# aswanthabam/JPEG_Decoder

Measured on AMD Instinct MI355X. Metric: Mpixels/s decoded (IDCT+colour), higher is better.
Workload: dtype f32; 1 GPU; stream of 4096x4096 baseline 4:4:4 images, 32 images per step (one launch) per GPU, coefficient blocks resident in HBM; sampling=4:4:4, parallelism=images sharded x1, no collective, launched_by=bench.py

## Files before the change

### jpeg_decoder_amd/csrc/jb_huff.hip

```cpp
#include <hip/hip_runtime.h>
#include <stdint.h>

#include "jb_huff_core.h"
#include "jb_kernels.h"

extern __shared__ __attribute__((aligned(16))) uint8_t lds[];

namespace {

constexpr uint32_t L = kJbhLanes;
constexpr int kMaxPasses = (int)L + 4;

__constant__ uint8_t kZz2Dev[64] = {0,   2,   16,  32,  18,  4,   6,   20,  34,  48, 64,  50,  36,  22,  8,   10,
                                    24,  38,  52,  66,  80,  96,  82,  68,  54,  40, 26,  12,  14,  28,  42,  56,
                                    70,  84,  98,  112, 114, 100, 86,  72,  58,  44, 30,  46,  60,  74,  88,  102,
                                    116, 118, 104, 90,  76,  62,  78,  92,  106, 120, 122, 108, 94,  110, 124, 126};

struct Misc {
  uint32_t *w;
  static constexpr uint32_t kBytes = 256u, kZz2 = 0u, kZz2Words = 64u / 4u, kScan = 16u, kScanWords = L / 64u * 5u, kFold = 40u, kFoldWords = 8u;
  static_assert(kZz2 + kZz2Words <= kScan && kScan + kScanWords <= kFold && (kFold + kFoldWords) * 4u <= kBytes, "sub-areas: disjoint, inside the 256 bytes");
  __device__ uint32_t *zz2() const { return w + kZz2; }
  __device__ uint32_t *scan() const { return w + kScan; }
  __device__ uint32_t *fold() const { return w + kFold; }
};
template <uint32_t kMaxChunk>
struct Lay {
  static constexpr uint32_t kRows = jbh_rows(kMaxChunk);
  static constexpr uint32_t kNcp = kMaxChunk * 8u / kJbCheckpointBits;
  static_assert(kNcp <= kJbCheckpoints, "records per chunk");
  static constexpr uint32_t off_cp = kRows * L * 4u;
  static constexpr uint32_t off_xbit = off_cp + kNcp * L * 4u;
  static constexpr uint32_t off_xmeta = off_xbit + L * 4u;
  static constexpr uint32_t off_misc = off_xmeta + L * 4u;
  static constexpr uint32_t off_tab = off_misc + Misc::kBytes;
  static constexpr uint32_t bytes(uint32_t n_tabs) { return off_tab + n_tabs * kJbT1Entries * 2u + kJbT2Tables * kJbT2Entries * 2u; }
  static __device__ uint32_t *stream() { return (uint32_t *)lds; }
  static __device__ uint32_t *cp() { return (uint32_t *)(lds + off_cp); }
  static __device__ uint32_t *xbit() { return (uint32_t *)(lds + off_xbit); }
  static __device__ uint32_t *xmeta() { return (uint32_t *)(lds + off_xmeta); }
  static __device__ Misc misc() { return Misc{(uint32_t *)(lds + off_misc)}; }
  static __device__ uint16_t *tab() { return (uint16_t *)(lds + off_tab); }
};
static_assert(Lay<64>::bytes(2) == 30976 && Lay<64>::bytes(3) == 33024 && Lay<64>::bytes(4) == 35072 && Lay<64>::bytes(5) == 37120 && Lay<64>::bytes(6) == 39168, "LDS bytes: 1.1 KiB more per workgroup cost a third of the waves (NOTES.md)");
static_assert(Lay<128>::bytes(2) == 49408 && Lay<128>::bytes(3) == 51456 && Lay<128>::bytes(4) == 53504 && Lay<128>::bytes(5) == 55552 && Lay<128>::bytes(6) == 57600, "LDS bytes");

struct LaneId {
  uint32_t ci;
  bool owned, active;
  uint32_t gidx;
  uint32_t start, end;
  uint32_t seg;
  bool first, last;
  uint32_t u0, u_end;
};
__device__ __forceinline__ LaneId lane_id(const JbHuffLaunch &p, const JbHuffImage &img, const JbHuffWg &wg, uint32_t tid, uint32_t warm, bool warm_go) {
  LaneId x;
  x.ci = wg.first_chunk + tid - warm;
  const bool has = tid < warm + kJbOwnChunks && x.ci < img.n_chunks;
  x.owned = tid >= warm && has;
  x.active = has && (x.owned || warm_go);
  x.gidx = img.state_off + (has ? x.ci : img.n_chunks - 1u);
  const JbChunkDesc cd = p.chunks[x.gidx];
  x.seg = cd.seg & 0x7fffffffu;
  x.first = (cd.seg >> 31) != 0;
  uint32_t seg_end = p.starts[img.int_off + x.seg + 1];
  if (seg_end > img.scan_len) seg_end = img.scan_len;
  x.start = cd.start < seg_end ? cd.start : seg_end;
  x.end = x.start + img.chunk_bytes < seg_end ? x.start + img.chunk_bytes : seg_end;
  x.last = x.end == seg_end;
  x.u0 = jbh_u_of_bit(x.start, x.start * 8u), x.u_end = x.u0 + (x.end - x.start) * 8u;
  return x;
}

template <uint32_t kRows>
__device__ __forceinline__ void load_stream(uint32_t *stream, const uint8_t *img_scan, uint32_t start, uint32_t tid) {
  const uint8_t *src = img_scan + (int32_t)jbh_base_byte(start);
#pragma unroll
  for (uint32_t q = 0; q < (kRows + 3u) / 4u; q++) {
    const uint4 v = *(const uint4 *)(src + 16u * q);
    const uint32_t d[4] = {v.x, v.y, v.z, v.w};
#pragma unroll
    for (uint32_t i = 0; i < 4; i++)
      if (4u * q + i < kRows) stream[(4u * q + i) * L + tid] = __builtin_bswap32(d[i]);
  }
}

__device__ __forceinline__ void load_tables(uint16_t *tab, const JbHuffLaunch &p, const JbHuffImage &img, uint32_t tid) {
  const JbHuffTables *set = p.tables + img.table_set;
  const uint4 *s1 = (const uint4 *)set->t1;
  uint4 *d = (uint4 *)tab;
  const uint32_t n1 = img.n_tabs * kJbT1Entries * 2u / 16u;
  for (uint32_t i = tid; i < n1; i += L) d[i] = s1[i];
  const uint4 *s2 = (const uint4 *)set->t2;
  constexpr uint32_t n2 = kJbT2Tables * kJbT2Entries * 2u / 16u;
  for (uint32_t i = tid; i < n2; i += L) d[n1 + i] = s2[i];
}

struct Seg {
  uint32_t f, n, d0, d1, d2;
};
__device__ __forceinline__ Seg seg_combine(const Seg &a, const Seg &b) {
  Seg r;
  r.f = a.f | b.f;
  r.n = b.f ? b.n : a.n + b.n;
  r.d0 = b.f ? b.d0 : a.d0 + b.d0;
  r.d1 = b.f ? b.d1 : a.d1 + b.d1;
  r.d2 = b.f ? b.d2 : a.d2 + b.d2;
  return r;
}
__device__ __forceinline__ Seg seg_shfl_up(const Seg &x, int off) {
  Seg r;
  r.f = __shfl_up(x.f, off);
  r.n = __shfl_up(x.n, off);
  r.d0 = __shfl_up(x.d0, off);
  r.d1 = __shfl_up(x.d1, off);
  r.d2 = __shfl_up(x.d2, off);
  return r;
}
__device__ __forceinline__ void seg_store(uint32_t *s, const Seg &x) { s[0] = x.f, s[1] = x.n, s[2] = x.d0, s[3] = x.d1, s[4] = x.d2; }
__device__ __forceinline__ Seg seg_load(const uint32_t *s) { return Seg{s[0], s[1], s[2], s[3], s[4]}; }
__device__ __forceinline__ Seg seg_scan_wg(Seg x, uint32_t *scratch, uint32_t tid, Seg *total) {
  const uint32_t lane = tid & 63u, wave = tid >> 6;
#pragma unroll
  for (int off = 1; off < 64; off <<= 1) {
    const Seg t = seg_shfl_up(x, off);
    if (lane >= (uint32_t)off) x = seg_combine(t, x);
  }
  __syncthreads();
  if (lane == 63u) seg_store(scratch + wave * 5u, x);
  __syncthreads();
  Seg run{0, 0, 0, 0, 0};
  Seg all{0, 0, 0, 0, 0};
#pragma unroll
  for (uint32_t w = 0; w < L / 64u; w++) {
    const Seg t = seg_load(scratch + w * 5u);
    if (w < wave) run = seg_combine(run, t);
    all = seg_combine(all, t);
  }
  *total = all;
  return seg_combine(run, x);
}

__device__ __forceinline__ Seg seg_left_workgroups(const JbHuffLaunch &p, const JbHuffImage &img, const JbHuffWg &wg, const Misc &misc, uint32_t tid) {
  const uint32_t w_first = img.wg0, w_me = img.wg0 + wg.first_chunk / kJbOwnChunks;
  uint32_t *const red = misc.fold();
  if (tid < 8) red[tid] = 0;
  __syncthreads();
  uint32_t last_f = 0;
  for (uint32_t w = w_first + tid; w < w_me; w += L)
    if (p.wgsum[w].has_first) last_f = w - w_first + 1u;
  if (last_f) atomicMax(&red[0], last_f);
  __syncthreads();
  const uint32_t from = red[0];
  uint32_t a_n = 0, a0 = 0, a1 = 0, a2 = 0;
  for (uint32_t w = w_first + tid; w < w_me; w += L) {
    if (w - w_first + 1u >= from) {
      const JbWgSum s = p.wgsum[w];
      a_n += s.blocks, a0 += s.dc[0], a1 += s.dc[1], a2 += s.dc[2];
    }
  }
  if (a_n) atomicAdd(&red[1], a_n);
  if (a0) atomicAdd(&red[2], a0);
  if (a1) atomicAdd(&red[3], a1);
  if (a2) atomicAdd(&red[4], a2);
  __syncthreads();
  return Seg{from ? 1u : 0u, red[1], red[2], red[3], red[4]};
}
__device__ __forceinline__ Seg seg_left_lanes(const Seg &mine, const Misc &misc, uint32_t tid) {
  Seg total;
  const Seg incl = seg_scan_wg(mine, misc.scan(), tid, &total);
  Seg left = seg_shfl_up(incl, 1);
  if ((tid & 63u) == 0) {
    left = Seg{0, 0, 0, 0, 0};
    for (uint32_t w = 0; w < (tid >> 6); w++) left = seg_combine(left, seg_load(misc.scan() + w * 5u));
  }
  return left;
}
__device__ __forceinline__ JbWgSum *wgsum_of(const JbHuffLaunch &p, const JbHuffImage &img, const JbHuffWg &wg) { return p.wgsum + img.wg0 + wg.first_chunk / kJbOwnChunks; }

}

template <uint32_t kMaxChunk>
__global__ __launch_bounds__(kJbHuffLanes) void jb_huff_sync_kernel(const JbHuffLaunch p, const int launch) {
  using Ly = Lay<kMaxChunk>;
  uint32_t *const xbit = Ly::xbit(), *const xmeta = Ly::xmeta();
  const uint32_t tid = threadIdx.x;
  const JbHuffWg wg = p.sync_wgs[blockIdx.x];
  const JbHuffImage img = p.images[wg.image];
  const LaneId me = lane_id(p, img, wg, tid, kJbWarmChunks, launch == 0);
  const size_t n_all = p.n_chunks_total;

  JbChunkState entry{me.start * 8u, 0u}, exitst{0u, 0u};
  bool changed = me.active;
  if (launch > 0) {
    bool c0 = false;
    JbChunkState ne{0u, 0u};
    if (tid == kJbWarmChunks && me.owned && !me.first) {
      ne = p.exit[me.gidx - 1u];
      c0 = !jbh_same_state(ne, p.entry[me.gidx]);
    }
    if (!__syncthreads_or(c0)) return;
    entry = p.entry[me.gidx];
    exitst = p.exit[me.gidx];
    changed = c0;
    if (c0) entry = jbh_entry_from_exit(ne);
  }
  load_tables(Ly::tab(), p, img, tid);
  if (me.active) load_stream<Ly::kRows>(Ly::stream(), p.scan + img.scan_off, me.start, tid);
  uint32_t *const cpl = Ly::cp() + tid;
#pragma unroll
  for (uint32_t i = 0; i < Ly::kNcp; i++) cpl[i * L] = launch > 0 ? p.cps[i * n_all + me.gidx] : kJbhCpNone;
  __syncthreads();
  const JbhCtx cx = jbh_ctx(Ly::stream() + tid, Ly::tab(), nullptr, img);

  for (int pass = 0; pass < kMaxPasses; pass++) {
    if (__builtin_amdgcn_ballot_w64(changed) != 0) {
      JbhLane st = jbh_lane_from(entry, me.start, me.u_end, cx.nb4, changed);
      uint32_t none = 0;
      while (st.u < me.u_end) {
        const uint32_t up = st.u;
        (void)jbh_step<false>(cx, st, none, none, none, nullptr, 0u);
        if (((st.u ^ up) >> 8) != 0) {
          uint32_t *rec = cpl + ((st.u >> 8) - 1u) * L;
          const uint32_t s = jbh_pack_state(st), old = *rec;
          const bool met = (st.u < me.u_end) & jbh_cp_same_place(old, s);
          *rec = met ? old : s;
          st.u = met ? jbh_met_at((st.u >> 8) - 1u) : st.u;
        }
      }
      JBH_TRACE_PASS_END(pass);
      if (changed) {
        if (jbh_has_met(st.u)) {
          const uint32_t met_i = jbh_met_checkpoint(st.u);
          const uint32_t dn = st.nblk - jbh_cp_blocks(cpl[met_i * L]);
          for (uint32_t i = met_i; i < Ly::kNcp; i++) cpl[i * L] = jbh_cp_add_blocks(cpl[i * L], dn);
          exitst.meta = jbh_meta_add_blocks(exitst.meta, dn);
        } else {
          exitst = JbChunkState{jbh_bit_of_u(me.start, st.u), jbh_exit_meta(st)};
        }
      }
    }
    xbit[tid] = exitst.bitpos;
    xmeta[tid] = jbh_meta_state(exitst.meta);
    __syncthreads();
    changed = false;
    if (me.active && !me.first && tid > (launch == 0 ? 0u : kJbWarmChunks)) {
      const uint32_t nbit = xbit[tid - 1u], nmeta = xmeta[tid - 1u];
      if (nbit != entry.bitpos || nmeta != jbh_meta_state(entry.meta)) {
        entry = JbChunkState{nbit, nmeta};
        changed = true;
      }
    }
    if (!__syncthreads_or(changed)) break;
  }
  if (me.owned) {
    p.entry[me.gidx] = entry;
    p.exit[me.gidx] = exitst;
#pragma unroll
    for (uint32_t i = 0; i < Ly::kNcp; i++) p.cps[i * n_all + me.gidx] = cpl[i * L];
  }
  Seg mine{0, 0, 0, 0, 0};
  if (me.owned) {
    mine.f = me.first ? 1u : 0u;
    mine.n = jbh_meta_blocks(exitst.meta) + (me.first ? me.seg * img.ri * img.nb : 0u);
  }
  Seg total;
  (void)seg_scan_wg(mine, Ly::misc().scan(), tid, &total);
  if (tid == 0) wgsum_of(p, img, wg)->has_first = total.f, wgsum_of(p, img, wg)->blocks = total.n;
}

template <uint32_t kMaxChunk>
__global__ __launch_bounds__(kJbHuffLanes) void jb_huff_write_kernel(const JbHuffLaunch p) {
  using Ly = Lay<kMaxChunk>;
  const Misc misc = Ly::misc();
  const uint32_t tid = threadIdx.x;
  const JbHuffWg wg = p.wgs[blockIdx.x];
  const JbHuffImage img = p.images[wg.image];
  const LaneId me = lane_id(p, img, wg, tid, 0u, false);
  const uint32_t bpi = img.ri * img.nb;

  load_tables(Ly::tab(), p, img, tid);
  if (tid < Misc::kZz2Words) misc.zz2()[tid] = ((const uint32_t *)kZz2Dev)[tid];
  if (me.active) load_stream<Ly::kRows>(Ly::stream(), p.scan + img.scan_off, me.start, tid);

  uint32_t err = 0;
  JbChunkState entry{me.start * 8u, 0u}, want{0u, 0u};
  uint32_t block = me.seg * bpi;
  if (img.needs_sync) {
    Seg mine{0, 0, 0, 0, 0};
    if (me.active) {
      want = p.exit[me.gidx];
      mine.f = me.first ? 1u : 0u;
      mine.n = jbh_meta_blocks(want.meta) + (me.first ? me.seg * bpi : 0u);
      if (!me.first) {
        const JbChunkState prev = p.exit[me.gidx - 1u];
        const JbChunkState en = p.entry[me.gidx];
        entry = JbChunkState{prev.bitpos, jbh_meta_state(prev.meta)};
        if (en.bitpos != prev.bitpos || jbh_meta_state(en.meta ^ prev.meta) != 0) err |= kJbStatusNotInStep;
      }
    }
    const Seg left = seg_combine(seg_left_workgroups(p, img, wg, misc, tid), seg_left_lanes(mine, misc, tid));
    if (!me.first) block = left.n;
  }
  __syncthreads();
  const JbhCtx cx = jbh_ctx(Ly::stream() + tid, Ly::tab(), (const uint8_t *)misc.zz2(), img);

  uint32_t block_end = (me.seg + 1u) * img.ri < img.n_mcus ? (me.seg + 1u) * bpi : img.n_mcus * img.nb;
  if (block_end > img.n_blocks) block_end = img.n_blocks;
  JbhLane st;
  const bool overran = me.active && entry.bitpos > me.end * 8u;
  {
    const uint32_t bit = entry.bitpos < me.start * 8u ? me.start * 8u : entry.bitpos;
    const uint32_t u = jbh_u_of_bit(me.start, bit);
    st.u = u < me.u_end ? u : me.u_end;
    st.k = entry.meta & kJbhMetaFieldMask;
    st.blk4 = ((entry.meta >> kJbhMetaBlkShift) & kJbhMetaFieldMask) * 4u;
    if (st.k > 63u) st.k = 0;
    if (st.blk4 >= cx.nb4) st.blk4 = 0;
    st.nblk = 0;
  }
  const uint32_t k_in = st.k;
  uint32_t dc0 = 0, dc1 = 0, dc2 = 0;
  uint8_t *const coef = (uint8_t *)p.coef + img.coef_off;
  bool live = me.active && st.u < me.u_end && block < block_end;
  while (live) {
    if (jbh_step<true>(cx, st, dc0, dc1, dc2, coef, block)) {
      err |= kJbStatusCorrupt;
      live = false;
    } else {
      live = st.u < me.u_end && block + st.nblk < block_end;
    }
  }
  JBH_TRACE_PASS_END(0);
  if (me.active) {
    if (me.last) {
      if (block + st.nblk != block_end || st.k != 0 || st.u > me.u_end || overran) err |= kJbStatusOverrun;
    } else if (img.needs_sync) {
      if (jbh_bit_of_u(me.start, st.u) != want.bitpos || jbh_exit_meta(st) != want.meta) err |= kJbStatusNotInStep;
    }
    if (err) atomicOr(p.status + wg.image, err);
    JbChunkDc o;
    o.dc[0] = dc0, o.dc[1] = dc1, o.dc[2] = dc2;
    o.first_block = block + (k_in != 0 ? 1u : 0u);
    o.count = err ? 0u : st.nblk + (st.k != 0 ? 1u : 0u) - (k_in != 0 ? 1u : 0u);
    o.pad[0] = o.pad[1] = o.pad[2] = 0;
    p.chunk_dc[me.gidx] = o;
  }
  if (img.needs_sync) {
    Seg mine{0, 0, 0, 0, 0};
    if (me.active) mine = Seg{me.first ? 1u : 0u, 0u, dc0, dc1, dc2};
    Seg total;
    (void)seg_scan_wg(mine, misc.scan(), tid, &total);
    if (tid == 0) {
      JbWgSum *o = wgsum_of(p, img, wg);
      o->dc[0] = total.d0, o->dc[1] = total.d1, o->dc[2] = total.d2;
    }
  }
}

__global__ __launch_bounds__(kJbHuffLanes) void jb_huff_dc_kernel(const JbHuffLaunch p) {
  const Misc misc{(uint32_t *)lds};
  const uint32_t tid = threadIdx.x;
  const JbHuffWg wg = p.wgs[blockIdx.x];
  const JbHuffImage img = p.images[wg.image];
  const LaneId me = lane_id(p, img, wg, tid, 0u, false);
  JbChunkDc cd = p.chunk_dc[me.gidx];
  if (!me.active) cd.count = 0;
  uint32_t p0 = 0, p1 = 0, p2 = 0;
  if (img.needs_sync) {
    Seg mine{0, 0, 0, 0, 0};
    if (me.active) mine = Seg{me.first ? 1u : 0u, 0u, cd.dc[0], cd.dc[1], cd.dc[2]};
    const Seg left = seg_combine(seg_left_workgroups(p, img, wg, misc, tid), seg_left_lanes(mine, misc, tid));
    if (!me.first) p0 = left.d0, p1 = left.d1, p2 = left.d2;
  }
  uint8_t *const coef = (uint8_t *)p.coef + img.coef_off;
  uint32_t pos4 = (cd.first_block % img.nb) * 4u;
  uint32_t bad = 0;
  constexpr uint32_t kBatch = 24;
  for (uint32_t i = 0; i < cd.count; i += kBatch) {
    int32_t diff[kBatch];
#pragma unroll
    for (uint32_t q = 0; q < kBatch; q++) diff[q] = i + q < cd.count ? *(const int16_t *)(coef + (size_t)jbh_mul24(cd.first_block + i + q, img.blk_bytes)) : 0;
#pragma unroll
    for (uint32_t q = 0; q < kBatch; q++) {
      if (i + q < cd.count) {
        const uint32_t c = jbh_ubfe(img.lut_comp, pos4, 4);
        const uint32_t pr = (c == 0 ? p0 : c == 1 ? p1 : p2) + (uint32_t)diff[q];
        bad |= (pr + 32768u) > 65535u ? 1u : 0u;
        p0 = c == 0 ? pr : p0;
        p1 = c == 1 ? pr : p1;
        p2 = c == 2 ? pr : p2;
        *(int16_t *)(coef + (size_t)jbh_mul24(cd.first_block + i + q, img.blk_bytes)) = (int16_t)pr;
        pos4 = pos4 + 4u == img.nb * 4u ? 0u : pos4 + 4u;
      }
    }
  }
  if (bad) atomicOr(p.status + wg.image, kJbStatusCorrupt);
}

__global__ __launch_bounds__(256) void jb_huff_fetch_kernel(uint4 *dst, const uint4 *src, uint32_t n16) {
  for (uint32_t i = blockIdx.x * 256u + threadIdx.x; i < n16; i += gridDim.x * 256u) dst[i] = src[i];
}
__global__ __launch_bounds__(256) void jb_huff_zero_kernel(uint4 *dst, uint64_t n16, uint4 *small, uint32_t small16) {
  const uint4 z = make_uint4(0, 0, 0, 0);
  if (blockIdx.x == 0 && threadIdx.x < small16) small[threadIdx.x] = z;
  for (uint64_t i = (uint64_t)blockIdx.x * 256u + threadIdx.x; i < n16; i += (uint64_t)gridDim.x * 256u) dst[i] = z;
}
hipError_t jbk_huff_zero(void *d_dst, size_t bytes, hipStream_t stream, void *d_small, size_t small_bytes) {
  (void)hipGetLastError();
  const uint64_t n16 = (bytes + 15) / 16;
  uint64_t blocks = (n16 + 255u) / 256u;
  if (blocks > 8192u) blocks = 8192u;
  const uint32_t small16 = d_small ? (uint32_t)((small_bytes + 15) / 16) : 0u;
  if (small16 > 256u) return hipErrorInvalidValue;
  hipLaunchKernelGGL(jb_huff_zero_kernel, dim3((unsigned)(blocks ? blocks : 1u)), dim3(256), 0, stream, (uint4 *)d_dst, n16, (uint4 *)d_small, small16);
  return hipGetLastError();
}
hipError_t jbk_huff_fetch(void *d_dst, const void *h_pinned_src, size_t bytes, hipStream_t stream) {
  (void)hipGetLastError();
  const uint32_t n16 = (uint32_t)((bytes + 15) / 16);
  unsigned blocks = (n16 + 255u) / 256u;
  if (blocks > 1024u) blocks = 1024u;
  hipLaunchKernelGGL(jb_huff_fetch_kernel, dim3(blocks ? blocks : 1u), dim3(256), 0, stream, (uint4 *)d_dst, (const uint4 *)h_pinned_src, n16);
  return hipGetLastError();
}

template <uint32_t kMaxChunk>
static void huff_launch(const JbHuffLaunch &p, hipStream_t stream) {
  const dim3 block(kJbHuffLanes);
  const uint32_t n_tabs = p.max_tabs < 2u ? 2u : p.max_tabs > kJbMaxTabs ? kJbMaxTabs : p.max_tabs;
  const unsigned lds_bytes = Lay<kMaxChunk>::bytes(n_tabs);
  if (p.n_sync_wgs > 0) {
    const int launches = p.sync_launches > 0 ? p.sync_launches : kJbSyncLaunches;
    for (int l = 0; l < launches; l++) hipLaunchKernelGGL(jb_huff_sync_kernel<kMaxChunk>, dim3((unsigned)p.n_sync_wgs), block, lds_bytes, stream, p, l);
  }
  if (p.n_wgs > 0) {
    hipLaunchKernelGGL(jb_huff_write_kernel<kMaxChunk>, dim3((unsigned)p.n_wgs), block, lds_bytes, stream, p);
    hipLaunchKernelGGL(jb_huff_dc_kernel, dim3((unsigned)p.n_wgs), block, Misc::kBytes, stream, p);
  }
}
hipError_t jbk_huff_launch(const JbHuffLaunch &p, hipStream_t stream) {
  (void)hipGetLastError();
  if (p.max_chunk_bytes <= 64u) huff_launch<64>(p, stream);
  else huff_launch<128>(p, stream);
  return hipGetLastError();
}
```

### jpeg_decoder_amd/csrc/jb_huff_core.h

```cpp
#pragma once
#include <stdint.h>

#include "jb_huff.h"

#if defined(__HIPCC__)
#define JBH_FN __host__ __device__ inline __attribute__((always_inline))
#else
#define JBH_FN inline
#endif

JBH_FN uint32_t jbh_alignbit(uint32_t hi, uint32_t lo, uint32_t sh) {
#if defined(__HIP_DEVICE_COMPILE__)
  return __builtin_amdgcn_alignbit(hi, lo, sh);
#else
  return (uint32_t)(((((uint64_t)hi) << 32) | lo) >> (sh & 31u));
#endif
}
JBH_FN uint32_t jbh_ubfe(uint32_t v, uint32_t off, uint32_t width) {
#if defined(__HIP_DEVICE_COMPILE__)
  return __builtin_amdgcn_ubfe(v, off, width);
#else
  off &= 31u, width &= 31u;
  return width ? (v >> off) & ((1u << width) - 1u) : 0u;
#endif
}
JBH_FN int32_t jbh_sbfe(uint32_t v, uint32_t off, uint32_t width) {
#if defined(__HIP_DEVICE_COMPILE__)
  return __builtin_amdgcn_sbfe((int32_t)v, off, width);
#else
  off &= 31u, width &= 31u;
  if (!width) return 0;
  const uint32_t f = (v >> off) & ((1u << width) - 1u);
  return (int32_t)(f << (32u - width)) >> (32u - width);
#endif
}

JBH_FN uint32_t jbh_mul24(uint32_t a, uint32_t b) { return (a & 0xffffffu) * (b & 0xffffffu); }

#ifndef JBH_TRACE_STEP
#define JBH_TRACE_STEP() ((void)0)
#define JBH_TRACE_PASS_END(pass) ((void)0)
#endif

constexpr uint32_t kJbhLanes = (uint32_t)kJbHuffLanes;
constexpr uint32_t jbh_rows(uint32_t chunk_bytes) { return chunk_bytes / 4u + 3u; }

JBH_FN uint32_t jbh_base_byte(uint32_t start) { return (start & ~3u) - 4u; }
JBH_FN uint32_t jbh_u_of_bit(uint32_t start, uint32_t bit) { return bit - 8u * jbh_base_byte(start) - 1u; }
JBH_FN uint32_t jbh_bit_of_u(uint32_t start, uint32_t u) { return u + 8u * jbh_base_byte(start) + 1u; }

struct JbhCtx {
  const uint32_t *scol;
  const uint16_t *tab;
  const uint8_t *zz2;
  uint32_t lut_ac, lut_dc, lut_comp;
  uint32_t nb4;
  uint32_t blk_bytes;
  uint32_t t2_first;
};
struct JbhLane {
  uint32_t u;
  uint32_t k;
  uint32_t blk4;
  uint32_t nblk;
};
JBH_FN JbhCtx jbh_ctx(const uint32_t *scol, const uint16_t *tab, const uint8_t *zz2, const JbHuffImage &img) {
  return JbhCtx{scol, tab, zz2, img.lut_ac, img.lut_dc, img.lut_comp, img.nb * 4u, img.blk_bytes, img.n_tabs * kJbT1Entries};
}

template <bool kStore>
JBH_FN bool jbh_step(const JbhCtx &cx, JbhLane &st, uint32_t &dc0, uint32_t &dc1, uint32_t &dc2, uint8_t *coef, uint32_t block0) {
  JBH_TRACE_STEP();
  const uint32_t u = st.u;
  const uint32_t j = jbh_ubfe(u, 5, 27);
  const uint32_t w = jbh_alignbit(cx.scol[j * kJbhLanes], cx.scol[j * kJbhLanes + kJbhLanes], ~u);
  const bool isdc = st.k == 0;
  const uint32_t tix = jbh_ubfe(isdc ? cx.lut_dc : cx.lut_ac, st.blk4, 4);
  uint32_t e = cx.tab[(tix << kJbT1Bits) + (w >> (32 - kJbT1Bits))];
  if (e - 1u < 31u)
    e = cx.tab[cx.t2_first + ((e - 1u) << kJbT2Bits) + ((w >> 16) & (kJbT2Entries - 1u))];
  const uint32_t total = e & 31u, size = (e >> 5) & 15u, adv = e >> 9;
  const uint32_t k1 = st.k + adv;
  const bool bad = e == 0 || (k1 - 65u) < 17u;
  if (kStore) {
    const int32_t x = jbh_sbfe(w, 32u - total, size);
    const int32_t val = x - (int32_t)(((1u << size) - 1u) ^ (uint32_t)(x >> 31));
    const uint32_t c = jbh_ubfe(cx.lut_comp, st.blk4, 4);
    const uint32_t dcv = (isdc && !bad) ? (uint32_t)val : 0u;
    dc0 += c == 0 ? dcv : 0u;
    dc1 += c == 1 ? dcv : 0u;
    dc2 += c == 2 ? dcv : 0u;
    if (!bad && (isdc || size != 0))
      *(int16_t *)(coef + (jbh_mul24(block0 + st.nblk, cx.blk_bytes) + cx.zz2[k1 - 1u])) = (int16_t)val;
  }
  const uint32_t k2 = k1 - ((size == 0 && !isdc) ? 1u : 0u);
  const bool done = k2 >= 64u;
  const bool next = done || bad;
  st.k = next ? 0u : k2;
  st.nblk += (done && !bad) ? 1u : 0u;
  const uint32_t b4 = st.blk4 + (next ? 4u : 0u);
  st.blk4 = b4 == cx.nb4 ? 0u : b4;
  st.u = u + (bad ? 1u : total);
  return bad;
}

constexpr uint32_t kJbhMetaBlkShift = 8, kJbhMetaFieldMask = 0xffu;
constexpr uint32_t kJbhMetaStateMask = 0xffffu, kJbhMetaCountShift = 16, kJbhMetaCountMask = 0xffffu;
JBH_FN uint32_t jbh_exit_meta(const JbhLane &st) { return st.k | (st.blk4 << (kJbhMetaBlkShift - 2u)) | ((st.nblk & kJbhMetaCountMask) << kJbhMetaCountShift); }
JBH_FN uint32_t jbh_meta_state(uint32_t meta) { return meta & kJbhMetaStateMask; }
JBH_FN uint32_t jbh_meta_blocks(uint32_t meta) { return meta >> kJbhMetaCountShift; }
JBH_FN uint32_t jbh_meta_add_blocks(uint32_t meta, uint32_t dn) { return (meta & kJbhMetaStateMask) | ((((meta >> kJbhMetaCountShift) + dn) & kJbhMetaCountMask) << kJbhMetaCountShift); }
JBH_FN bool jbh_same_state(const JbChunkState &a, const JbChunkState &b) { return a.bitpos == b.bitpos && ((a.meta ^ b.meta) & kJbhMetaStateMask) == 0; }
JBH_FN JbChunkState jbh_entry_from_exit(const JbChunkState &x) { return JbChunkState{x.bitpos, x.meta & kJbhMetaStateMask}; }
JBH_FN JbhLane jbh_lane_from(const JbChunkState &entry, uint32_t start, uint32_t u_end, uint32_t nb4, bool go) {
  const uint32_t u = jbh_u_of_bit(start, entry.bitpos < start * 8u ? start * 8u : entry.bitpos);
  const uint32_t k = entry.meta & kJbhMetaFieldMask, blk4 = ((entry.meta >> kJbhMetaBlkShift) & kJbhMetaFieldMask) * 4u;
  return JbhLane{(go && u < u_end) ? u : u_end, k > 63u ? 0u : k, blk4 >= nb4 ? 0u : blk4, 0u};
}

constexpr uint32_t kJbhCpKShift = 11, kJbhCpBlk4Shift = 15, kJbhCpCountShift = 20, kJbhCpPlaceMask = 0xfffffu, kJbhCpNone = 0xffffffffu;
JBH_FN uint32_t jbh_pack_state(const JbhLane &st) { return st.u | (st.k << kJbhCpKShift) | (st.blk4 << kJbhCpBlk4Shift) | (st.nblk << kJbhCpCountShift); }
JBH_FN bool jbh_cp_same_place(uint32_t a, uint32_t b) { return ((a ^ b) & kJbhCpPlaceMask) == 0; }
JBH_FN uint32_t jbh_cp_blocks(uint32_t rec) { return rec >> kJbhCpCountShift; }
JBH_FN uint32_t jbh_cp_add_blocks(uint32_t rec, uint32_t dn) { return rec + (dn << kJbhCpCountShift); }
constexpr uint32_t kJbhMet = 0x80000000u, kJbhMetIndexMask = 0xffu;
JBH_FN uint32_t jbh_met_at(uint32_t checkpoint) { return kJbhMet | checkpoint; }
JBH_FN bool jbh_has_met(uint32_t u) { return u >= kJbhMet; }
JBH_FN uint32_t jbh_met_checkpoint(uint32_t u) { return u & kJbhMetIndexMask; }

#include <string.h>

inline uint16_t jbh_entry_(bool is_ac, int len, int sym) {
  if (!is_ac) {
    if (sym > 11) return 0;
    return (uint16_t)((len + sym) | (sym << 5) | (1 << 9));
  }
  const int run = sym >> 4, size = sym & 15;
  if (size > 10) return 0;
  if (sym == 0) return (uint16_t)(len | (kJbAdvEob << 9));
  if (sym == 0xf0) return (uint16_t)(len | (17 << 9));
  return (uint16_t)((len + size) | (size << 5) | ((run + 1) << 9));
}

inline bool jb_huff_fill_table_impl_(const uint8_t counts[17], const uint8_t *symbols, bool is_ac, JbHuffTables *set, uint32_t tix, uint32_t n_tabs,
                                     uint32_t *n_t2) {
  uint16_t *t1 = set->t1[tix];
  memset(t1, 0, sizeof set->t1[0]);
  uint32_t code = 0;
  int k = 0;
  int32_t sub_of_prefix = -1;
  uint32_t sub_prefix = 0;
  for (int len = 1; len <= 16; len++) {
    for (int i = 0; i < counts[len]; i++, k++, code++) {
      if (code >= (1u << len)) return false;
      const uint16_t e = jbh_entry_(is_ac, len, symbols[k]);
      if (len <= kJbT1Bits) {
        const uint32_t first = code << (kJbT1Bits - len);
        for (uint32_t q = 0; q < (1u << (kJbT1Bits - len)); q++) t1[first + q] = e;
      } else {
        const uint32_t prefix = code >> (len - kJbT1Bits);
        if (sub_of_prefix < 0 || sub_prefix != prefix) {
          if (*n_t2 >= kJbT2Tables) return false;
          sub_of_prefix = (int32_t)(*n_t2)++;
          sub_prefix = prefix;
          memset(set->t2[sub_of_prefix], 0, sizeof set->t2[0]);
          t1[prefix] = (uint16_t)(sub_of_prefix + 1);
        }
        const uint32_t rest = len - kJbT1Bits;
        const uint32_t first = (code & ((1u << rest) - 1u)) << (kJbT2Bits - rest);
        for (uint32_t q = 0; q < (1u << (kJbT2Bits - rest)); q++) set->t2[sub_of_prefix][first + q] = e;
      }
    }
    code <<= 1;
  }
  return true;
}
```

Before: 629,500 Mpixels/s.

## Compact live Huffman sync lanes per checkpoint segment to cut wave divergence

```diff
diff --git a/jpeg_decoder_amd/csrc/jb_huff.hip b/jpeg_decoder_amd/csrc/jb_huff.hip
--- a/jpeg_decoder_amd/csrc/jb_huff.hip
+++ b/jpeg_decoder_amd/csrc/jb_huff.hip
@@ -33,17 +33,20 @@
   static constexpr uint32_t off_xbit = off_cp + kNcp * L * 4u;
   static constexpr uint32_t off_xmeta = off_xbit + L * 4u;
   static constexpr uint32_t off_misc = off_xmeta + L * 4u;
-  static constexpr uint32_t off_tab = off_misc + Misc::kBytes;
+  static constexpr uint32_t off_list = off_misc + Misc::kBytes;
+  static constexpr uint32_t off_tab = off_list + L;
   static constexpr uint32_t bytes(uint32_t n_tabs) { return off_tab + n_tabs * kJbT1Entries * 2u + kJbT2Tables * kJbT2Entries * 2u; }
   static __device__ uint32_t *stream() { return (uint32_t *)lds; }
   static __device__ uint32_t *cp() { return (uint32_t *)(lds + off_cp); }
   static __device__ uint32_t *xbit() { return (uint32_t *)(lds + off_xbit); }
   static __device__ uint32_t *xmeta() { return (uint32_t *)(lds + off_xmeta); }
   static __device__ Misc misc() { return Misc{(uint32_t *)(lds + off_misc)}; }
+  static __device__ uint8_t *list() { return lds + off_list; }
   static __device__ uint16_t *tab() { return (uint16_t *)(lds + off_tab); }
 };
-static_assert(Lay<64>::bytes(2) == 30976 && Lay<64>::bytes(3) == 33024 && Lay<64>::bytes(4) == 35072 && Lay<64>::bytes(5) == 37120 && Lay<64>::bytes(6) == 39168, "LDS bytes: 1.1 KiB more per workgroup cost a third of the waves (NOTES.md)");
-static_assert(Lay<128>::bytes(2) == 49408 && Lay<128>::bytes(3) == 51456 && Lay<128>::bytes(4) == 53504 && Lay<128>::bytes(5) == 55552 && Lay<128>::bytes(6) == 57600, "LDS bytes");
+static_assert(Lay<64>::bytes(2) == 31232 && Lay<64>::bytes(3) == 33280 && Lay<64>::bytes(4) == 35328 && Lay<64>::bytes(5) == 37376 && Lay<64>::bytes(6) == 39424, "LDS bytes: 1.1 KiB more per workgroup cost a third of the waves (NOTES.md)");
+static_assert(Lay<128>::bytes(2) == 49664 && Lay<128>::bytes(3) == 51712 && Lay<128>::bytes(4) == 53760 && Lay<128>::bytes(5) == 55808 && Lay<128>::bytes(6) == 57856, "LDS bytes");
+static_assert(Lay<128>::bytes(4) <= 54613, "three workgroups per CU with four tables: 160 KiB / 3");
 
 struct LaneId {
   uint32_t ci;
@@ -181,6 +184,13 @@
 
 }
 
+__device__ __forceinline__ JbChunkState state_load(const JbChunkState *q) {
+  const uint64_t v = __atomic_load_n((const uint64_t *)q, __ATOMIC_RELAXED);
+  return JbChunkState{(uint32_t)v, (uint32_t)(v >> 32)};
+}
+__device__ __forceinline__ void state_store(JbChunkState *q, const JbChunkState &s) { __atomic_store_n((uint64_t *)q, (uint64_t)s.bitpos | ((uint64_t)s.meta << 32), __ATOMIC_RELAXED); }
+static_assert(sizeof(JbChunkState) == 8, "one 64-bit access (the arrays are 16-byte aligned: jb_huff_pack_)");
+
 template <uint32_t kMaxChunk>
 __global__ __launch_bounds__(kJbHuffLanes) void jb_huff_sync_kernel(const JbHuffLaunch p, const int launch) {
   using Ly = Lay<kMaxChunk>;
@@ -197,12 +207,12 @@
     bool c0 = false;
     JbChunkState ne{0u, 0u};
     if (tid == kJbWarmChunks && me.owned && !me.first) {
-      ne = p.exit[me.gidx - 1u];
-      c0 = !jbh_same_state(ne, p.entry[me.gidx]);
+      ne = state_load(p.exit + (me.gidx - 1u));
+      c0 = !jbh_same_state(ne, state_load(p.entry + me.gidx));
     }
     if (!__syncthreads_or(c0)) return;
-    entry = p.entry[me.gidx];
-    exitst = p.exit[me.gidx];
+    entry = state_load(p.entry + me.gidx);
+    exitst = state_load(p.exit + me.gidx);
     changed = c0;
     if (c0) entry = jbh_entry_from_exit(ne);
   }
@@ -212,33 +222,81 @@
 #pragma unroll
   for (uint32_t i = 0; i < Ly::kNcp; i++) cpl[i * L] = launch > 0 ? p.cps[i * n_all + me.gidx] : kJbhCpNone;
   __syncthreads();
-  const JbhCtx cx = jbh_ctx(Ly::stream() + tid, Ly::tab(), nullptr, img);
-
+  JbhCtx cx = jbh_ctx(Ly::stream(), Ly::tab(), nullptr, img);
+
+  const uint32_t wave = tid >> 6;
+  uint8_t *const list = Ly::list();
+  uint32_t *const n_live = Ly::misc().scan();
+  uint32_t turn = 0;
   for (int pass = 0; pass < kMaxPasses; pass++) {
-    if (__builtin_amdgcn_ballot_w64(changed) != 0) {
-      JbhLane st = jbh_lane_from(entry, me.start, me.u_end, cx.nb4, changed);
-      uint32_t none = 0;
-      while (st.u < me.u_end) {
-        const uint32_t up = st.u;
-        (void)jbh_step<false>(cx, st, none, none, none, nullptr, 0u);
-        if (((st.u ^ up) >> 8) != 0) {
-          uint32_t *rec = cpl + ((st.u >> 8) - 1u) * L;
-          const uint32_t s = jbh_pack_state(st), old = *rec;
-          const bool met = (st.u < me.u_end) & jbh_cp_same_place(old, s);
-          *rec = met ? old : s;
-          st.u = met ? jbh_met_at((st.u >> 8) - 1u) : st.u;
+    uint32_t c = tid, round = 0;
+    bool live = changed;
+    const bool dense = launch == 0 && pass == 0;
+#pragma unroll 1
+    for (; round < Ly::kNcp + 2u; round++) {
+      const uint64_t m = __builtin_amdgcn_ballot_w64(live);
+      if (live) list[wave * 64u + __builtin_amdgcn_mbcnt_hi((uint32_t)(m >> 32), __builtin_amdgcn_mbcnt_lo((uint32_t)m, 0u))] = (uint8_t)c;
+      if ((tid & 63u) == 0) n_live[turn + wave] = (uint32_t)__builtin_popcountll(m);
+      __syncthreads();
+      const uint32_t n0 = n_live[turn], n1 = n0 + n_live[turn + 1u], n2 = n1 + n_live[turn + 2u], n3 = n2 + n_live[turn + 3u];
+      turn ^= 4u;
+      if (n3 == 0) break;
+      const bool work = tid < n3;
+      if (work) {
+        const uint32_t w = (tid >= n0 ? 1u : 0u) + (tid >= n1 ? 1u : 0u) + (tid >= n2 ? 1u : 0u);
+        c = list[w * 64u + tid - (w == 0 ? 0u : w == 1 ? n0 : w == 2 ? n1 : n2)];
+      }
+      if (round == 0 && changed) {
+        const JbhLane s0 = jbh_lane_from(entry, me.start, me.u_end, cx.nb4, true);
+        xbit[tid] = jbh_pack_state(s0), xmeta[tid] = me.u_end;
+      }
+      __syncthreads();
+      live = false;
+      if (__builtin_amdgcn_ballot_w64(work) != 0) {
+        JbhLane st{0u, 0u, 0u, 0u};
+        uint32_t u_end = 0;
+        if (work) st = jbh_unpack_state(xbit[c]), u_end = xmeta[c] & kJbhTaskEndMask;
+        const uint32_t u_from = st.u, u_next = (st.u | 255u) + 1u, u_stop = u_next < u_end ? u_next : u_end;
+        cx.scol = Ly::stream() + c;
+        uint32_t none = 0;
+        if (dense) {
+          while (st.u < u_end) {
+            const uint32_t up = st.u;
+            (void)jbh_step<false>(cx, st, none, none, none, nullptr, 0u);
+            if (((st.u ^ up) >> 8) != 0) Ly::cp()[c + ((st.u >> 8) - 1u) * L] = jbh_pack_state(st);
+          }
+        } else {
+          while (st.u < u_stop) (void)jbh_step<false>(cx, st, none, none, none, nullptr, 0u);
         }
-      }
-      JBH_TRACE_PASS_END(pass);
-      if (changed) {
-        if (jbh_has_met(st.u)) {
-          const uint32_t met_i = jbh_met_checkpoint(st.u);
-          const uint32_t dn = st.nblk - jbh_cp_blocks(cpl[met_i * L]);
-          for (uint32_t i = met_i; i < Ly::kNcp; i++) cpl[i * L] = jbh_cp_add_blocks(cpl[i * L], dn);
-          exitst.meta = jbh_meta_add_blocks(exitst.meta, dn);
-        } else {
-          exitst = JbChunkState{jbh_bit_of_u(me.start, st.u), jbh_exit_meta(st)};
+        JBH_TRACE_PASS_END(pass);
+        if (work) {
+          uint32_t flags = u_end;
+          if (!dense && ((st.u ^ u_from) >> 8) != 0) {
+            const uint32_t i = (st.u >> 8) - 1u;
+            uint32_t *rec = Ly::cp() + c + i * L;
+            const uint32_t s = jbh_pack_state(st), old = *rec;
+            const bool met = (st.u < u_end) & jbh_cp_same_place(old, s);
+            *rec = met ? old : s;
+            flags |= met ? kJbhTaskMet | (i << kJbhTaskMetShift) : 0u;
+          }
+          live = st.u < u_end && (flags & kJbhTaskMet) == 0;
+          xbit[c] = jbh_pack_state(st), xmeta[c] = flags | (live ? kJbhTaskLive : 0u);
         }
+      } else {
+        JBH_TRACE_PASS_END(pass);
+      }
+    }
+    if (round == 0) break;
+    if (changed) {
+      const JbhLane st = jbh_unpack_state(xbit[tid]);
+      const uint32_t flags = xmeta[tid];
+      if (flags & kJbhTaskMet) {
+        const uint32_t met_i = flags >> kJbhTaskMetShift;
+        const uint32_t dn = st.nblk - jbh_cp_blocks(cpl[met_i * L]);
+        for (uint32_t i = met_i; i < Ly::kNcp; i++) cpl[i * L] = jbh_cp_add_blocks(cpl[i * L], dn);
+        exitst.meta = jbh_meta_add_blocks(exitst.meta, dn);
+      } else {
+        exitst = JbChunkState{jbh_bit_of_u(me.start, st.u), jbh_exit_meta(st)};
       }
     }
     xbit[tid] = exitst.bitpos;
@@ -252,11 +310,10 @@
         changed = true;
       }
     }
-    if (!__syncthreads_or(changed)) break;
   }
   if (me.owned) {
-    p.entry[me.gidx] = entry;
-    p.exit[me.gidx] = exitst;
+    state_store(p.entry + me.gidx, entry);
+    state_store(p.exit + me.gidx, exitst);
 #pragma unroll
     for (uint32_t i = 0; i < Ly::kNcp; i++) p.cps[i * n_all + me.gidx] = cpl[i * L];
   }
diff --git a/jpeg_decoder_amd/csrc/jb_huff_core.h b/jpeg_decoder_amd/csrc/jb_huff_core.h
--- a/jpeg_decoder_amd/csrc/jb_huff_core.h
+++ b/jpeg_decoder_amd/csrc/jb_huff_core.h
@@ -123,6 +123,10 @@
 JBH_FN bool jbh_cp_same_place(uint32_t a, uint32_t b) { return ((a ^ b) & kJbhCpPlaceMask) == 0; }
 JBH_FN uint32_t jbh_cp_blocks(uint32_t rec) { return rec >> kJbhCpCountShift; }
 JBH_FN uint32_t jbh_cp_add_blocks(uint32_t rec, uint32_t dn) { return rec + (dn << kJbhCpCountShift); }
+JBH_FN JbhLane jbh_unpack_state(uint32_t rec) {
+  return JbhLane{rec & ((1u << kJbhCpKShift) - 1u), (rec >> kJbhCpKShift) & 63u, (rec >> kJbhCpBlk4Shift) & 0x1cu, rec >> kJbhCpCountShift};
+}
+constexpr uint32_t kJbhTaskEndMask = 0xffffu, kJbhTaskLive = 1u << 16, kJbhTaskMet = 1u << 17, kJbhTaskMetShift = 24;
 constexpr uint32_t kJbhMet = 0x80000000u, kJbhMetIndexMask = 0xffu;
 JBH_FN uint32_t jbh_met_at(uint32_t checkpoint) { return kJbhMet | checkpoint; }
 JBH_FN bool jbh_has_met(uint32_t u) { return u >= kJbhMet; }
```

Measured after the change: 629,100 Mpixels/s. About the same (-0.1%).
